# crabml/crabml

Measured on NVIDIA H100. Metric: decode_tokens_per_s, higher is better.
Workload: dtype int8

## Files before the change

crabml_b200/csrc/common.cuh:

```cuda
#pragma once

#include <cuda_fp16.h>
#include <cuda_runtime.h>
#include <stdint.h>

#include <atomic>
#include <map>
#include <mutex>
#include <set>
#include <string>
#include <unordered_map>
#include <vector>

#include "../../include/crabml_cuda.h"

#define QK_K 256

#define CC_D_STRIDE(nb) ((((nb) + 7) / 8) * 8)
#define CC_HAS_PADDED_D(t) ((t) == CC_Q8_0 || (t) == CC_Q4_0)
#define CC_MAX_PLANES 4
#define CC_N_SLOTS 16
#define CC_HISTORY_CAP 65536

struct cc_device;
// ... 182 lines not shown
    const uint8_t* p3[3];
    float* out[3];
    int m[3];
    int n;
};
struct StreamArgs {
    StreamMats mats;
    const void* act;
    int k;
    int epilogue;
    const float* residual;
    const uint16_t* exp_lut;
};
struct AttnArgs {
    const float *q, *k, *v;
    void *kcache, *vcache;
    float* out;
    void* act_scratch;
    const int64_t* dyn;
    const float* rope_tab;
    int n_heads, n_kv, hd, rope_dim, max_len, kv_f16;
    int64_t seq_stride;
    float scale;
};
struct DeqPlanes { const uint8_t* p[CC_MAX_PLANES]; int64_t cols; };
enum { MK_NORMQ = 0, MK_MATVEC = 1, MK_ATTN = 2, MK_ROWS = 3, MK_REDUCE = 4, MK_GATHER = 5, MK_ARGMAX = 6, MK_SAMPLE = 7 };
struct MkPhase {
    int type, wtype, write_back, next_matvec;
    int xgpu, red_n; const float* next_norm_w; float* red_dst; const float* red_res;
    float* x; float* orig; const float* norm_w; float eps; int n; ActQ8_0 act;
    int act_type, next_norm_n;
    StreamArgs mv;
    AttnArgs at;
    unsigned long long dyn_off, rope_off;
    DeqPlanes planes; int src_dtype, dst_dtype, n_rows, pad; long long cols; void* dst;
    const long long* rows_dev;
    long long* slot_dev; long long* hist_dev;
    int norm_ahead, pad2;
};
#define MK_PROF_SLOTS 9
size_t cc_mega_smem_for_phase(const MkPhase& ph);
const CommDev* cc_comm_dev(cc_device* dev);
bool cc_comm_is_nccl(cc_device* dev);
int cc_comm_world(cc_device* dev);
void cc_comm_destroy(cc_device* dev);
int cc_launch_all_reduce(cc_device* dev, float* x, int64_t n, const float* residual);
int cc_launch_all_gather(cc_device* dev, const float* src, int64_t n, float* dst);
extern "C" CC_API int cc_test_mega_barrier_floor(cc_device* dev, int n, float* us_per_phase);
enum MegaVariant { MEGA_NONE = 0, MEGA_REGISTER = 1, MEGA_RING = 2 };
struct MegaLaunch {
    MegaVariant variant = MEGA_NONE;
    size_t smem = 1024, wstage = 0;
    int slot_bytes = 0, nslots = 0, at_ch = 64;
    bool generic = false, sample = false;
};
int cc_launch_mega(cc_device* dev, const MkPhase* phases_dev, int n_phases, const uint8_t* dyn_dev, unsigned* bar_dev, const MegaLaunch& L,
                   unsigned long long* prof);
bool cc_mega_test_stall();
bool cc_mega_ring_phase_ok(const MkPhase& ph);
int cc_mega_ring_at_ch(const MkPhase& ph);
size_t cc_mega_ring_smem_for_phase(const MkPhase& ph);
int cc_mega_ring_slots(const MegaLaunch& L);
int cc_launch_mega_ring(cc_device* dev, const MkPhase* phases_dev, int n_phases, const uint8_t* dyn_dev, unsigned* bar_dev, const MegaLaunch& L,
                        unsigned long long* prof, const CommDev* comm);
int cc_check_async_error(cc_device* dev);
int cc_launch_normq(cc_device* dev, float* x, float* orig, const float* norm_w, float eps, int64_t n, void* act_scratch, bool write_back);
int cc_launch_attn_decode(cc_device* dev, const AttnArgs& a);
bool cc_attn_decode_fits(int64_t hd, int64_t max_len);
struct LazyState;
LazyState* cc_lazy_create(cc_device* dev);
void cc_lazy_destroy(cc_device* dev);
int cc_lazy_flush(cc_device* dev);
int cc_lazy_invalidate(cc_device* dev);
bool cc_stream_supported(int type, int64_t k);
bool cc_mega_generic_supported(int type, int64_t k);
int cc_launch_matvec_stream(cc_device* dev, int type, const StreamArgs& A);
int cc_launch_matvec_stream_plain(cc_device* dev, const cc_buf* w, const void* act, float* out, int64_t m, int64_t k);
// ... 90 lines not shown
```

crabml_b200/csrc/lazy.cu:

```cuda
#include <math.h>
#include <stdlib.h>
#include <string.h>

#include <chrono>
#include <functional>

#include "sample_dev.cuh"

enum LKind { L_COPY_ROWS, L_DUP, L_RMS_NORM, L_MUL, L_ADD, L_SCALE, L_MATVEC, L_ROPE, L_CONCAT, L_CONTIGUOUS, L_BMM, L_SOFTMAX, L_SILU, L_GELU, L_ALLREDUCE, L_ALLGATHER, L_ARGMAX, L_SAMPLE };

struct LView { cc_buf* buf = nullptr; int ndim = 0; int64_t shape[CC_MAX_DIMS] = {0, 0, 0, 0}, strides[CC_MAX_DIMS] = {0, 0, 0, 0}; };

struct LOp {
    int kind;
    LView a, b;
    cc_buf* out = nullptr;
    float f = 0.0f;
    int64_t i0 = 0, i1 = 0, i2 = 0;
    std::vector<int64_t> rows;
    bool done = false;
};

struct GraphEntry { cudaGraphExec_t exec = nullptr; size_t dyn_bytes = 0; uint64_t launches = 0; MkPhase* phases_dev = nullptr;
                    std::vector<uint64_t> sig; uint64_t last_use = 0; MegaVariant mega_variant = MEGA_NONE; };
#define LZ_MAX_GRAPHS 64

struct LazyState {
    std::vector<LOp> q;
    std::unordered_map<cc_buf*, int> qrefs;
#define LZ_DYN_SLOTS 8
    uint8_t* dyn_host[LZ_DYN_SLOTS] = {nullptr};
    cudaEvent_t dyn_ev[LZ_DYN_SLOTS] = {nullptr};
    int dyn_slot = 0;
    uint8_t* dyn_dev = nullptr;
    size_t dyn_cap = 1 << 16;
    void* act[2] = {nullptr, nullptr};
    unsigned* bar_dev = nullptr;
    unsigned long long* prof_dev = nullptr;
    std::vector<int> prof_types;
    size_t act_cap = 0;
    std::unordered_map<uint64_t, GraphEntry> cache;
    uint64_t flushes = 0, graph_hits = 0, captures = 0, uncached = 0, evictions = 0, collisions = 0;
    uint64_t ns_record = 0, ns_fuse = 0, ns_submit = 0, n_ops = 0;
    MegaVariant mega_variant = MEGA_NONE;
};

static LView mkview(const cc_view* v) {
    LView l;
    if (!v) return l;
    l.buf = v->buf; l.ndim = v->ndim;
    for (int i = 0; i < v->ndim; i++) { l.shape[i] = v->shape[i]; l.strides[i] = v->strides[i]; }
    return l;
}
static int64_t vlen(const LView& v) { int64_t n = 1; for (int i = 0; i < v.ndim; i++) n *= v.shape[i]; return n; }
static bool vcontig(const LView& v) {
    if (v.ndim == 0) return true;
    if (v.strides[v.ndim - 1] != 1) return false;
    int64_t last = 1;
    for (int i = v.ndim - 1; i >= 0; i--) { if (last != v.strides[i]) return false; last *= v.shape[i]; }
// ... 4 lines not shown
    if (ge.exec) cudaGraphExecDestroy(ge.exec);
    if (ge.phases_dev) cudaFree(ge.phases_dev);
    ge.exec = nullptr; ge.phases_dev = nullptr;
}
static void graph_cache_clear(LazyState* lz) {
    for (auto& kv : lz->cache) graph_entry_free(kv.second);
    lz->cache.clear();
}
int cc_lazy_invalidate(cc_device* dev) {
    LazyState* lz = dev->lz;
    if (!lz) return CC_OK;
    graph_cache_clear(lz);
    if (cudaMemsetAsync(lz->bar_dev, 0, 4096, dev->stream) != cudaSuccess) return cc_fail(dev, CC_ERR_CUDA, "lazy: barrier reset failed");
    return CC_OK;
}

LazyState* cc_lazy_create(cc_device* dev) {
    LazyState* lz = new LazyState();
    for (int i = 0; i < LZ_DYN_SLOTS; i++)
        if (cudaMallocHost(&lz->dyn_host[i], lz->dyn_cap) != cudaSuccess || cudaEventCreateWithFlags(&lz->dyn_ev[i], cudaEventDisableTiming) != cudaSuccess) { delete lz; return nullptr; }
    if (cudaMalloc(&lz->dyn_dev, lz->dyn_cap) != cudaSuccess) { delete lz; return nullptr; }
    if (getenv("CRABML_MEGA_PROF") && cudaMalloc(&lz->prof_dev, MK_PROF_SLOTS * 8 * 4097) == cudaSuccess) cudaMemset(lz->prof_dev, 0, MK_PROF_SLOTS * 8 * 4097);
    if (cudaMalloc(&lz->bar_dev, 4096) != cudaSuccess || cudaMemset(lz->bar_dev, 0, 4096) != cudaSuccess) { delete lz; return nullptr; }
    return lz;
}
void cc_lazy_destroy(cc_device* dev) {
    LazyState* lz = dev->lz;
    if (!lz) return;
    for (auto& op : lz->q) { if (op.a.buf) cc_tensor_release(op.a.buf); if (op.b.buf) cc_tensor_release(op.b.buf); if (op.out) cc_tensor_release(op.out); }
    for (auto& kv : lz->cache) graph_entry_free(kv.second);
    lz->cache.clear();
    if (lz->bar_dev) cudaFree(lz->bar_dev);
    for (int i = 0; i < LZ_DYN_SLOTS; i++) { if (lz->dyn_host[i]) cudaFreeHost(lz->dyn_host[i]); if (lz->dyn_ev[i]) cudaEventDestroy(lz->dyn_ev[i]); }
    if (lz->dyn_dev) cudaFree(lz->dyn_dev);
    for (int i = 0; i < 2; i++) if (lz->act[i]) cudaFree(lz->act[i]);
    delete lz;
    dev->lz = nullptr;
}

static void hold(LazyState* lz, cc_buf* b) { if (b) { cc_tensor_retain(b); lz->qrefs[b]++; } }

int cc_lazy_record(cc_device* dev, int kind, const cc_view* a, const cc_view* b, cc_buf* out, float f, int64_t i0, int64_t i1, int64_t i2,
                   const int64_t* rows, int n_rows) {
    LazyState* lz = dev->lz;
    auto t0 = std::chrono::steady_clock::now();
    LOp op;
    op.kind = kind; op.a = mkview(a); op.b = mkview(b); op.out = out; op.f = f; op.i0 = i0; op.i1 = i1; op.i2 = i2;
    if (rows) op.rows.assign(rows, rows + n_rows);
    hold(lz, op.a.buf); hold(lz, op.b.buf); hold(lz, op.out);
    lz->q.push_back(std::move(op));
    lz->n_ops++;
    lz->ns_record += (uint64_t)std::chrono::duration_cast<std::chrono::nanoseconds>(std::chrono::steady_clock::now() - t0).count();
    return CC_OK;
}

struct Plan {
    std::vector<uint64_t> sig;
    std::vector<uint8_t> dyn;
// ... 248 lines not shown
        if (!cc_attn_decode_fits(hd, seq_stride / hd)) return 0;
        if (!dead_after(ct.out, i + 9) || !dead_after(b1.out, i + 9) || !dead_after(qb, i + 9) || !dead_after(kb, i + 9) || !dead_after(vb, i + 9)) return 0;
        const int64_t pos = rq.i0, rope_dim = rq.rows[0];
        if (rope_dim > hd || rope_dim % 2) return 0;
        if (rope_off == (size_t)-1 || rope_pos != pos || rope_hd != hd || this->rope_dim != rope_dim) {
            std::vector<float> tab((size_t)rope_dim);
            const int pairs = (int)rope_dim / 2;
            float theta_scale = powf(10000.0f, -2.0f / (float)hd), theta = (float)pos;
            for (int j = 0; j < pairs; j++) { tab[j] = cosf(theta); tab[pairs + j] = sinf(theta); theta *= theta_scale; }
            rope_off = P.dyn_put(tab.data(), tab.size() * 4);
            rope_pos = pos; rope_hd = (int)hd; this->rope_dim = (int)rope_dim;
        }
        int64_t dynv[2] = {pos, kv_len};
        size_t dyn_off = P.dyn_put(dynv, sizeof(dynv));
        AttnArgs A = {};
        A.q = (const float*)qb->plane[0]; A.k = (const float*)kb->plane[0]; A.v = (const float*)vb->plane[0];
        A.kcache = kc->plane[0]; A.vcache = vc->plane[0];
        A.out = (float*)b2.out->base;
        if (*quantized && is(i + 9, L_MATVEC) && !cc_stream_supported(q[i + 9].a.buf->dtype, q[i + 9].a.shape[1])) *quantized = false;
        A.act_scratch = *quantized ? lz->act[1] : nullptr;
        A.n_heads = (int)n_heads; A.n_kv = (int)n_kv; A.hd = (int)hd; A.rope_dim = (int)rope_dim;
        A.max_len = (int)(seq_stride / hd); A.kv_f16 = kc->dtype == CC_F16;
        A.seq_stride = seq_stride; A.scale = sc.f;
        cc_device* d = dev;
        size_t roff = rope_off;
        P.S(0x2004); P.SP(A.q); P.SP(A.k); P.SP(A.v); P.SP(A.kcache); P.SP(A.vcache); P.SP(A.out); P.SP(A.act_scratch);
        P.S(n_heads); P.S(n_kv); P.S(hd); P.S(rope_dim); P.S(seq_stride); P.S(A.kv_f16); uint32_t sb; memcpy(&sb, &A.scale, 4); P.S(sb); P.S(dyn_off); P.S(roff);
        P.steps.push_back([=](uint8_t* dyn_dev) {
            AttnArgs B = A;
            B.dyn = (const int64_t*)(dyn_dev + dyn_off);
            B.rope_tab = (const float*)(dyn_dev + roff);
            return cc_launch_attn_decode(d, B);
        });
        { MkPhase ph = {}; ph.type = MK_ATTN; ph.at = A; ph.dyn_off = dyn_off; ph.rope_off = roff; ph.act = cc_act_q8_0(lz->act[1], n_heads * hd);
          P.phases.push_back(ph); }
        *obuf = b2.out;
        for (size_t t = i; t < i + 9; t++) q[t].done = true;
        return 9;
    }

    size_t try_copy_rows(size_t i) {
        if (!is(i, L_COPY_ROWS)) return 0;
        const LOp& op = q[i];
        cc_device* d = dev;
        const cc_buf* src = op.b.buf;
        void* dst = op.a.buf->plane[0];
        int dt = op.a.buf->dtype;
        int64_t cols = op.a.shape[op.a.ndim - 1];
        const int slot = (int)op.i2 - 1;
// ... 133 lines not shown
    }
};

static MegaLaunch choose_mega(const cc_device* dev, bool mega_ok, std::vector<MkPhase>& phs) {
    MegaLaunch L;
    if (!dev->mega || !mega_ok || phs.empty()) return L;
    bool stream = false, ring_ok = true;
    int n_sample = 0;
    for (auto& ph : phs) {
        if (ph.type == MK_MATVEC) (ph.act_type == CC_Q8_K ? L.generic : stream) = true;
        if (!cc_mega_ring_phase_ok(ph)) ring_ok = false;
        n_sample += ph.type == MK_SAMPLE;
    }
    L.sample = n_sample > 0;
    if (n_sample > 1 || (n_sample == 1 && phs.back().type != MK_SAMPLE)) return L;
    for (auto& ph : phs) {
        L.smem = std::max(L.smem, stream ? cc_mega_ring_smem_for_phase(ph) : cc_mega_smem_for_phase(ph));
        if (ph.type == MK_MATVEC && ph.x && ph.norm_w) L.wstage = std::max(L.wstage, (size_t)ph.n * 4);
        if (stream && ph.type == MK_MATVEC && ph.act_type != CC_Q8_K) L.slot_bytes = std::max(L.slot_bytes, ph.wtype == CC_Q8_0 ? 4352 : 2304);
        if (stream && ph.type == MK_ATTN) L.at_ch = cc_mega_ring_at_ch(ph);
    }
    if (stream ? !ring_ok || !(L.nslots = cc_mega_ring_slots(L)) : L.smem + L.wstage + 4096 > 227 * 1024) return L;
    L.variant = stream ? MEGA_RING : MEGA_REGISTER;
    int nxt = -1, nxn = -1;
    for (int t = (int)phs.size() - 1; t >= 0; t--) {
        MkPhase& ph = phs[t];
        ph.next_matvec = nxt;
        ph.next_norm_w = nxn >= 0 && phs[nxn].norm_ahead ? phs[nxn].norm_w : nullptr;
        ph.next_norm_n = ph.next_norm_w ? phs[nxn].n : 0;
        if (ph.type == MK_MATVEC) nxt = t;
        if (ph.type == MK_MATVEC && ph.x && ph.norm_w) nxn = t;
    }
    return L;
}

static int size_scratch(cc_device* dev, LazyState* lz) {
    int64_t max_k = 0;
    for (auto& op : lz->q) if (op.kind == L_MATVEC) max_k = std::max<int64_t>(max_k, std::max<int64_t>(op.a.shape[1], 0));
    for (auto& op : lz->q) if (op.kind == L_BMM && op.b.ndim == 3 && op.b.strides[2] == 1) max_k = std::max<int64_t>(max_k, op.a.shape[0] * op.b.shape[2]);
    size_t need = cc_act_bytes(CC_Q8_0, (max_k + 255) / 256 * 256) + 256;
    int rc = CC_OK;
    if (need > lz->act_cap) {
        cudaStreamSynchronize(dev->stream);
        graph_cache_clear(lz);
        for (int i = 0; i < 2; i++) { if (lz->act[i]) cudaFree(lz->act[i]); lz->act[i] = nullptr; }
        size_t cap = (size_t)1 << 20; while (cap < need) cap <<= 1;
        for (int i = 0; i < 2; i++) if (cudaMalloc(&lz->act[i], cap) != cudaSuccess) return cc_fail(dev, CC_ERR_CUDA, "lazy: scratch alloc failed");
        lz->act_cap = cap;
    }
    for (auto& op : lz->q) if (op.kind == L_MATVEC) {
        int at = cc_partner_type(op.a.buf->dtype);
        int64_t bb = op.b.ndim == 1 ? 1 : op.b.shape[0];
        if (at != CC_F32 && (rc = cc_ensure_act_scratch(dev, cc_act_bytes(at, bb * op.a.shape[1])))) return rc;
    }
    for (auto& op : lz->q) if (op.kind == L_SAMPLE && (rc = cc_ensure_sample_scratch(dev, vlen(op.a)))) return rc;
    return CC_OK;
}

static int upload_dyn(cc_device* dev, LazyState* lz, const Plan& P) {
    if (P.dyn.size() > lz->dyn_cap) return cc_fail(dev, CC_ERR_UNSUPPORTED, "lazy: dynamic argument block too large");
    if (P.dyn.empty()) return CC_OK;
    int rc = CC_OK; const int s = lz->dyn_slot;
    lz->dyn_slot = (s + 1) % LZ_DYN_SLOTS;
    cudaEventSynchronize(lz->dyn_ev[s]);
    memcpy(lz->dyn_host[s], P.dyn.data(), P.dyn.size());
    if (cudaMemcpyAsync(lz->dyn_dev, lz->dyn_host[s], P.dyn.size(), cudaMemcpyHostToDevice, dev->stream) != cudaSuccess) rc = cc_fail(dev, CC_ERR_CUDA, "lazy: dyn upload failed");
    cudaEventRecord(lz->dyn_ev[s], dev->stream);
    return rc;
}

static int run_steps(const Plan& P, uint8_t* dyn_dev) {
// ... 136 lines not shown
```

crabml_b200/csrc/mega.cu:

```cuda
#define MK_SYNC() __syncthreads()
#include "mega_phases.cuh"

struct MkNextNorm { const float* norm_w; int norm_n; };

template <bool SMP>
__global__ void __launch_bounds__(MK_THREADS, MK_CTAS_PER_SM) mega_kernel(const MkPhase* __restrict__ phases, int n_phases, const uint8_t* dyn,
                                                                         unsigned* bar, const uint16_t* exp_lut, unsigned long long* prof, bool test_stall, int wtop_off,
                                                                         unsigned* err_host) {
    extern __shared__ __align__(16) uint8_t smem[];
    __shared__ float s_red[MK_WARPS];
    __shared__ MkPhase s_phs[2];
    __shared__ MkNextNorm s_next;
    __shared__ int s_abort;
    __shared__ __align__(8) unsigned long long s_abar[AT_NBUF];
    unsigned apar = 0u;
    const unsigned abar0 = (unsigned)__cvta_generic_to_shared(&s_abar[0]);
    if (threadIdx.x == 0) { for (int i = 0; i < AT_NBUF; i++) mbar_init(abar0 + 8u * i, 1u); s_abort = 0; }
    asm volatile("fence.mbarrier_init.release.cluster;" ::: "memory");
    asm volatile("fence.proxy.async.shared::cta;" ::: "memory");
    __syncthreads();
    const CommDev nocomm = {};
    KSeg S0, S1;
    uint8_t* work = smem;
    float* s_w = (float*)(smem + wtop_off);
    int wstaged = -1;
    int xstaged = -1;
    unsigned gen = 0;
    if (threadIdx.x == MK_BAR_THREAD) gen = ld_acquire_u32(&bar[32]);
    {
        const int* src = (const int*)phases;
        int* dst = (int*)&s_phs[0];
// ... 9 lines not shown
        const int nx = s_ph.next_matvec;
        const bool look = nx > p && nx < n_phases;
        int desc_w = 0, next_w = 0;
        if (p + 1 < n_phases && threadIdx.x < sizeof(MkPhase) / 4) desc_w = ((const int*)(phases + p + 1))[threadIdx.x];
        if (look && threadIdx.x < 3) {
            const MkPhase* ph = phases + nx;
            next_w = threadIdx.x < 2 ? ((const int*)&ph->norm_w)[threadIdx.x] : ph->x && ph->norm_w && ph->norm_ahead ? ph->n : 0;
        }
        switch (s_ph.type) {
        case MK_NORMQ: phase_normq(s_ph, s_red); break;
        case MK_MATVEC: {
            unsigned long long* st1 = stamp ? prof + p * MK_PROF_SLOTS + 1 : nullptr;
            switch (s_ph.wtype) {
            case CC_Q2_K: phase_matvec_generic<TQ2_K>(s_ph, work, s_w, wstaged == p, xstaged == p, exp_lut, st1, S0, S1); break;
            case CC_Q3_K: phase_matvec_generic<TQ3_K>(s_ph, work, s_w, wstaged == p, xstaged == p, exp_lut, st1, S0, S1); break;
            case CC_Q4_K: phase_matvec_generic<TQ45_K<false>>(s_ph, work, s_w, wstaged == p, xstaged == p, exp_lut, st1, S0, S1); break;
            case CC_Q5_K: phase_matvec_generic<TQ45_K<true>>(s_ph, work, s_w, wstaged == p, xstaged == p, exp_lut, st1, S0, S1); break;
            case CC_Q6_K: phase_matvec_generic<TQ6_K>(s_ph, work, s_w, wstaged == p, xstaged == p, exp_lut, st1, S0, S1); break;
            default: phase_matvec_generic<TQ8_K>(s_ph, work, s_w, wstaged == p, xstaged == p, exp_lut, st1, S0, S1); break;
            }
            break;
        }
        case MK_ATTN:
            if (s_ph.at.kv_f16) phase_attn<true>(s_ph, (float*)work, s_red, dyn, exp_lut, abar0, apar, AT_CH); else phase_attn<false>(s_ph, (float*)work, s_red, dyn, exp_lut, abar0, apar, AT_CH);
            break;
        case MK_ROWS: phase_rows(s_ph, dyn); break;
        case MK_ARGMAX: phase_argmax(s_ph, dyn, s_red); break;
        }
        if (stamp) prof[p * MK_PROF_SLOTS + 2] = globaltimer_ns();
        if (p + 1 < n_phases && threadIdx.x < sizeof(MkPhase) / 4) ((int*)&s_phs[(p + 1) & 1])[threadIdx.x] = desc_w;
        if (look && threadIdx.x < 3) ((int*)&s_next)[threadIdx.x] = next_w;
        const bool more = p + 1 < n_phases;
        if (test_stall && p == 2 && blockIdx.x == gridDim.x - 1) { if (threadIdx.x == 0) s_abort = 1; break; }
        if (more) grid_barrier_arrive(bar, gridDim.x, gen);
        if (look && s_next.norm_n > 0) {
            const unsigned sw = (unsigned)__cvta_generic_to_shared(s_w);
            const float* nw = s_next.norm_w;
            for (int i = threadIdx.x; i < (s_next.norm_n >> 2); i += MK_THREADS)
                asm volatile("cp.async.cg.shared.global [%0], [%1], 16;" ::"r"(sw + i * 16), "l"(nw + i * 4) : "memory");
            asm volatile("cp.async.commit_group;" ::: "memory");
            wstaged = nx;
        }
        if (stamp) prof[p * MK_PROF_SLOTS + 3] = globaltimer_ns();
        if (more) {
            grid_barrier_wait(bar, gridDim.x, gen, nocomm, 0u, &s_abort, err_host);
            gen++;
            if (s_abort) break;
// ... 31 lines not shown
    CC_CUDA(dev, cudaMalloc(&d_tab, tab.size() * sizeof(MkPhase)));
    CC_CUDA(dev, cudaMalloc(&d_bar, 4096));
    CC_CUDA(dev, cudaMemcpy(d_tab, tab.data(), tab.size() * sizeof(MkPhase), cudaMemcpyHostToDevice));
    cudaEvent_t e0, e1;
    cudaEventCreate(&e0); cudaEventCreate(&e1);
    float best = 1e30f;
    for (int rep = 0; rep < 4; rep++) {
        CC_CUDA(dev, cudaMemsetAsync(d_bar, 0, 4096, dev->stream));
        cudaEventRecord(e0, dev->stream);
        MegaLaunch L;
        L.variant = MEGA_REGISTER;
        int rc = cc_launch_mega(dev, d_tab, n, nullptr, d_bar, L, nullptr);
        if (rc) return rc;
        cudaEventRecord(e1, dev->stream);
        CC_CUDA(dev, cudaEventSynchronize(e1));
        float ms = 0; cudaEventElapsedTime(&ms, e0, e1);
        if (ms < best) best = ms;
    }
    *us_per_phase = best * 1e3f / (float)n;
    cudaEventDestroy(e0); cudaEventDestroy(e1); cudaFree(d_tab); cudaFree(d_bar);
    return CC_OK;
}

bool cc_mega_generic_supported(int type, int64_t k) {
    return (type == CC_Q2_K || type == CC_Q3_K || type == CC_Q4_K || type == CC_Q5_K || type == CC_Q6_K || type == CC_Q8_K) && k % 256 == 0 && k <= 32768;
}

bool cc_mega_test_stall() {
    static const bool on = getenv("CRABML_MEGA_FLAGS") && (strtol(getenv("CRABML_MEGA_FLAGS"), nullptr, 0) & MK_F_TESTSTALL);
    return on;
}

int cc_launch_mega(cc_device* dev, const MkPhase* phases_dev, int n_phases, const uint8_t* dyn_dev, unsigned* bar_dev, const MegaLaunch& L,
                   unsigned long long* prof) {
    int max_ctas_per_sm = 0;
    const size_t wtop = (L.smem + 15) & ~(size_t)15;
    const size_t smem = wtop + L.wstage;
    CC_REQUIRE(dev, smem <= 227 * 1024, "megakernel: a phase needs %zu bytes of shared memory", smem);
    auto kern = L.sample ? mega_kernel<true> : mega_kernel<false>;
    if (smem > 48 * 1024) CC_CUDA(dev, cudaFuncSetAttribute(kern, cudaFuncAttributeMaxDynamicSharedMemorySize, (int)smem));
    CC_CUDA(dev, cudaOccupancyMaxActiveBlocksPerMultiprocessor(&max_ctas_per_sm, kern, MK_THREADS, smem));
    CC_REQUIRE(dev, max_ctas_per_sm >= 1, "megakernel does not fit on an SM");
    int per_sm = max_ctas_per_sm < MK_CTAS_PER_SM ? max_ctas_per_sm : MK_CTAS_PER_SM;
    const uint16_t* lut = dev->exp_lut;
    return mk_launch(dev, kern, dev->sm_count * per_sm, MK_THREADS, smem, phases_dev, n_phases, dyn_dev, bar_dev, lut, prof, cc_mega_test_stall(),
                     (int)wtop, dev->err_host);
}
```

crabml_b200/csrc/mega_phases.cuh:

```cuda
#pragma once
#include <stdlib.h>
#include <string.h>

#include "common.cuh"
#include "dequant.cuh"
#include "quantize_dev.cuh"
#include "vecdot.cuh"
#include "sample_dev.cuh"

#ifndef MK_SYNC
#error "define MK_SYNC() before including mega_phases.cuh"
#endif

#define MK_THREADS 512
#define MK_WARPS 16
#define MK_CTAS_PER_SM 1
#define MK_SEG 4
#define MK_XSTAGE_ROWS 512

__device__ __forceinline__ unsigned ld_acquire_u32(const unsigned* p) {
    unsigned v;
    asm volatile("ld.acquire.gpu.global.u32 %0, [%1];" : "=r"(v) : "l"(p) : "memory");
    return v;
}
// ... 234 lines not shown
        auto finish = [&]() { if (++c_seg < NSEG) return; c_seg = 0; const float v = warp_sum(acc); acc = 0.0f; emit(c_i++, v); };
        for (int u = 0; u < U; u += 2) {
            acc = T::seg_dot(S0, x0, k, c_seg, smem, lane, acc);
            finish();
            load(S0, x0, u + 2 < U);
            if (u + 1 >= U) break;
            acc = T::seg_dot(S1, x1, k, c_seg, smem, lane, acc);
            finish();
            load(S1, x1, u + 3 < U);
        }
    } else {
        for (int i = 0; i < n_vrows; i++) {
            int mat;
            const int r = locate(i, mat);
            emit(i, warp_sum(T::row_dot(planes(mat), r, k, smem, lane)));
        }
    }
    flush_pending();
}

#define AT_CH 64
#define AT_NBUF 3
template <bool KV_F16>
static __device__ void phase_attn(const MkPhase& ph, float* sm, float* s_red, const uint8_t* dyn, const uint16_t* exp_lut, unsigned abar0, unsigned& apar, const int at_ch) {
    const AttnArgs& a = ph.at;
    const int n_heads = a.n_heads, n_kv = a.n_kv, hd = a.hd, rope_dim = a.rope_dim;
    const int64_t seq_stride = a.seq_stride;
    const int64_t* dynv = (const int64_t*)(dyn + ph.dyn_off);
    const float* rope_tab = (const float*)(dyn + ph.rope_off);
    const int kv_len = (int)dynv[1], L = kv_len + 1;
    const int lane = threadIdx.x & 31, warp = threadIdx.x >> 5;
    float* s_q = sm; float* s_k = sm + hd; float* s_v = sm + 2 * hd; float* s_p = sm + 3 * hd;
    uint8_t* s_buf = (uint8_t*)(sm + 3 * hd + ((a.max_len + 8 + 3) & ~3));
    const unsigned s_buf_smem = (unsigned)__cvta_generic_to_shared(s_buf);
    constexpr int ELT = KV_F16 ? 2 : 4;
    const unsigned buf_bytes = (unsigned)(at_ch * hd * ELT);
    const int pairs = rope_dim >> 1;
    const int hd4 = hd >> 2;
    const int NC = (kv_len + at_ch - 1) / at_ch;
    auto issue_job = [&](int g, int j) {
        const int c = j < NC ? j : j - NC;
        const int p0 = c * at_ch, cnt = min(at_ch, kv_len - p0);
        const uint8_t* src = (const uint8_t*)(j < NC ? a.kcache : a.vcache) + ((int64_t)g * seq_stride + (int64_t)p0 * hd) * ELT;
        const unsigned bytes = (unsigned)(cnt * hd * ELT), bar = abar0 + 8u * (unsigned)(j % AT_NBUF), dst = s_buf_smem + (unsigned)(j % AT_NBUF) * buf_bytes;
        asm volatile("mbarrier.arrive.expect_tx.shared::cta.b64 _, [%0], %1;" ::"r"(bar), "r"(bytes) : "memory");
        asm volatile("cp.async.bulk.shared::cluster.global.mbarrier::complete_tx::bytes [%0], [%1], %2, [%3];" ::"r"(dst), "l"(src), "r"(bytes), "r"(bar) : "memory");
    };
// ... 101 lines not shown
            if (KV_F16) { acch = __hadd(acch, __hmul(__float2half_rn(s_v[d]), __float2half_rn(s_p[kv_len]))); o = __half2float(acch); }
            else { accf += s_p[kv_len] * s_v[d]; o = accf; }
            a.out[h * hd + d] = o;
            s_o[d] = o;
        }
        MK_SYNC();
        if (a.act_scratch) {
            ActQ8_0 act = ph.act;
            for (int b = warp; b < (hd >> 5); b += MK_WARPS) {
                float v = s_o[b * 32 + lane];
                float amax = warp_max(fabsf(v));
                float dd = amax / 127.0f;
                int qq = __float2int_rz(v / dd);
                const int gb = h * (hd >> 5) + b;
                act.qs[gb * 32 + lane] = (int8_t)qq;
                int ss = warp_sum_i(qq);
                if (lane == 0) { act.d[gb] = __half2float(__float2half_rn(dd)); act.isum[gb] = ss; }
            }
        }
        MK_SYNC();
    }
}

static __device__ void phase_rows(const MkPhase& ph, const uint8_t* dyn) {
    const int64_t* rows = ph.rows_dev ? (const int64_t*)ph.rows_dev : (const int64_t*)(dyn + ph.dyn_off);
    const int64_t total = (int64_t)ph.n_rows * ph.cols;
    for (int64_t i = (int64_t)blockIdx.x * MK_THREADS + threadIdx.x; i < total; i += (int64_t)gridDim.x * MK_THREADS) {
        const int64_t r = i / ph.cols, c = i - r * ph.cols;
        const int64_t e = rows[r] * ph.cols + c;
        float v;
        if (ph.src_dtype == CC_F32) v = __ldcg((const float*)ph.planes.p[0] + e);
        else if (ph.src_dtype == CC_F16) v = __half2float(((const __half*)ph.planes.p[0])[e]);
        else v = dequant_elem(ph.src_dtype, ph.planes, e);
        if (ph.dst_dtype == CC_F32) ((float*)ph.dst)[i] = v; else ((__half*)ph.dst)[i] = __float2half_rn(v);
    }
}

static __device__ void phase_argmax(const MkPhase& ph, const uint8_t* dyn, float* s_red) {
    if (blockIdx.x != 0) return;
    __shared__ long long s_idx[MK_WARPS];
    const float* x = ph.x;
    float bv = 0.0f; long long bi = -1;
    for (long long i = threadIdx.x; i < ph.n; i += MK_THREADS) { const float v = ldcg_f(x + i); if (bi < 0 || !(v < bv)) { bv = v; bi = i; } }
#pragma unroll
    for (int o = 16; o > 0; o >>= 1) {
        const float ov = __shfl_xor_sync(0xffffffffu, bv, o);
// ... 63 lines not shown
```

crabml_b200/csrc/mega_ring.cu:

```cuda
#define MK_SYNC() asm volatile("bar.sync 1, 512;" ::: "memory")
#define MK_GENERIC_NOINLINE 1
#include "mega_phases.cuh"

#define MR_PRODUCER_WARPS 4
#define MR_THREADS (MK_THREADS + 32 * MR_PRODUCER_WARPS)
#define MR_MAX_SLOTS 112
#define MR_Q8_SLOTS 24
#define MR_DESC_WORDS ((int)(sizeof(MkPhase) / 4))
#define MR_DESC_PER_LANE ((MR_DESC_WORDS + 31) / 32)

struct MrRing {
    int ring_off;
    int slot_bytes;
    int nslots;
    int at_ch;
};

__device__ __forceinline__ void mr_expect_tx(unsigned bar, unsigned bytes) { asm volatile("mbarrier.arrive.expect_tx.shared::cta.b64 _, [%0], %1;" ::"r"(bar), "r"(bytes) : "memory"); }
__device__ __forceinline__ void mr_bulk_g2s(unsigned dst, const void* src, unsigned bytes, unsigned bar, unsigned long long pol) {
    asm volatile("cp.async.bulk.shared::cluster.global.mbarrier::complete_tx::bytes.L2::cache_hint [%0], [%1], %2, [%3], %4;" ::"r"(dst), "l"(src), "r"(bytes), "r"(bar), "l"(pol) : "memory");
}
__device__ __forceinline__ void mr_stage_f32(float* dst, const float* src, int n) {
    const unsigned s = (unsigned)__cvta_generic_to_shared(dst);
    for (int i = threadIdx.x; i < (n >> 2); i += MK_THREADS) asm volatile("cp.async.cg.shared.global [%0], [%1], 16;" ::"r"(s + i * 16), "l"(src + i * 4) : "memory");
// ... 384 lines not shown
                    int mat;
                    const int rr = mr_locate(M, g, rc, 0, mat);
                    float* o = mat == 0 ? M.out[0] : mat == 1 ? M.out[1] : M.out[2];
                    o[rr] = r;
                }
            }
        }
    }
    flush_pending();
    if (stamp1) { stamp1[5] = (unsigned long long)c_wait; stamp1[6] = ((unsigned long long)(clock64() - c_all) << 20) | (unsigned long long)c_n; }
    RC.ent_base += (unsigned)(g.n_units * g.E);
    if (A.epilogue == 3) {
        MK_SYNC();
        if (warp < comm.world) {
            const size_t off = ((size_t)((xseq + 1u) & 1u) * CC_COMM_MAX_RANKS + comm.rank) * CC_COMM_MAX_ELEMS + g.first;
            for (int c4 = lane * 4; c4 < g.n_units; c4 += 128) *(float4*)(comm.data[warp] + off + c4) = *(const float4*)(s_part + c4);
        }
    }
}

template <bool GEN, bool SMP>
__global__ void __launch_bounds__(MR_THREADS, 1) mega_ring_kernel(const MkPhase* __restrict__ phases, int n_phases, const uint8_t* dyn, unsigned* bar,
                                                                  const uint16_t* exp_lut, unsigned long long* prof, bool test_stall, int wtop_off, unsigned* err_host,
                                                                  const CommDev comm, const MrRing R) {
    extern __shared__ __align__(128) uint8_t smem[];
    __shared__ float s_red[MK_WARPS];
    __shared__ MkPhase s_phs[2];
    __shared__ MkPhase s_pd[MR_PRODUCER_WARPS][2];
    __shared__ int s_abort;
    __shared__ int s_prod_done;
    __shared__ int s_ring_dead;
    __shared__ int s_unit;
    __shared__ __align__(8) unsigned long long s_abar[AT_NBUF];
    __shared__ __align__(8) unsigned long long s_full[MR_MAX_SLOTS];
    __shared__ unsigned s_done[MR_MAX_SLOTS];
    __shared__ unsigned s_seq[MR_MAX_SLOTS];
    unsigned apar = 0u;
    const unsigned abar0 = (unsigned)__cvta_generic_to_shared(&s_abar[0]);
    const unsigned full0 = (unsigned)__cvta_generic_to_shared(&s_full[0]);
    const unsigned done0 = (unsigned)__cvta_generic_to_shared(&s_done[0]);
    if (threadIdx.x == 0) {
        for (int i = 0; i < AT_NBUF; i++) mbar_init(abar0 + 8u * i, 1u);
        for (int i = 0; i < R.nslots; i++) { mbar_init(full0 + 8u * i, 1u); s_done[i] = 0u; s_seq[i] = 0u; }
        s_abort = 0; s_prod_done = 0; s_ring_dead = 0;
    }
    asm volatile("fence.mbarrier_init.release.cluster;" ::: "memory");
    asm volatile("fence.proxy.async.shared::cta;" ::: "memory");
// ... 24 lines not shown
        static_assert(sizeof(MkPhase) / 4 <= MK_THREADS, "descriptor does not fit one word per thread");
        int desc_w = 0;
        if (p + 1 < n_phases && threadIdx.x < sizeof(MkPhase) / 4) desc_w = ((const int*)(phases + p + 1))[threadIdx.x];
        unsigned long long* st1 = stamp ? prof + p * MK_PROF_SLOTS + 1 : nullptr;
        switch (s_ph.type) {
        case MK_NORMQ: phase_normq(s_ph, s_red); break;
        case MK_MATVEC:
            if (GEN && s_ph.act_type == CC_Q8_K) {
                switch (s_ph.wtype) {
                case CC_Q2_K: phase_matvec_generic<TQ2_K>(s_ph, work, s_wn, s_ph.norm_w == wst, false, exp_lut, st1); break;
                case CC_Q3_K: phase_matvec_generic<TQ3_K>(s_ph, work, s_wn, s_ph.norm_w == wst, false, exp_lut, st1); break;
                case CC_Q4_K: phase_matvec_generic<TQ45_K<false>>(s_ph, work, s_wn, s_ph.norm_w == wst, false, exp_lut, st1); break;
                case CC_Q5_K: phase_matvec_generic<TQ45_K<true>>(s_ph, work, s_wn, s_ph.norm_w == wst, false, exp_lut, st1); break;
                case CC_Q6_K: phase_matvec_generic<TQ6_K>(s_ph, work, s_wn, s_ph.norm_w == wst, false, exp_lut, st1); break;
                default: phase_matvec_generic<TQ8_K>(s_ph, work, s_wn, s_ph.norm_w == wst, false, exp_lut, st1); break;
                }
                if (s_ph.x && s_ph.norm_w) { wst = s_ph.next_norm_w; if (wst) mr_stage_f32(s_wn, wst, s_ph.next_norm_n); }
                break;
            }
            if (s_ph.wtype == CC_Q8_0) phase_matvec_ring<CC_Q8_0>(s_ph, work, s_wn, wst, xstaged == p, exp_lut, RC, comm, xseq, st1);
            else phase_matvec_ring<CC_Q4_0>(s_ph, work, s_wn, wst, xstaged == p, exp_lut, RC, comm, xseq, st1);
            break;
        case MK_ATTN:
            if (s_ph.at.kv_f16) phase_attn<true>(s_ph, (float*)work, s_red, dyn, exp_lut, abar0, apar, R.at_ch);
            else phase_attn<false>(s_ph, (float*)work, s_red, dyn, exp_lut, abar0, apar, R.at_ch);
            break;
        case MK_ROWS: phase_rows(s_ph, dyn); break;
        case MK_REDUCE: phase_reduce(s_ph, comm, xseq, false); break;
        case MK_GATHER: phase_reduce(s_ph, comm, xseq, true); break;
        case MK_ARGMAX: phase_argmax(s_ph, dyn, s_red); break;
        }
        if (stamp) prof[p * MK_PROF_SLOTS + 2] = globaltimer_ns();
        if (p + 1 < n_phases && threadIdx.x < sizeof(MkPhase) / 4) ((int*)&s_phs[(p + 1) & 1])[threadIdx.x] = desc_w;
        const bool more = p + 1 < n_phases;
        const bool xg = s_ph.xgpu != 0;
        if (test_stall && p == 2 && blockIdx.x == gridDim.x - 1) { if (threadIdx.x == 0) s_abort = 1; break; }
        if (more) grid_barrier_arrive(bar, gridDim.x, gen);
        if (stamp) prof[p * MK_PROF_SLOTS + 3] = globaltimer_ns();
        if (more) {
            grid_barrier_wait(bar, gridDim.x, gen, comm, xg ? xseq + 1u : 0u, &s_abort, err_host);
            gen++; if (xg) xseq++;
            if (s_abort) break;
            const MkPhase& nph = s_phs[(p + 1) & 1];
            if (nph.type == MK_MATVEC && nph.act_type != CC_Q8_K && nph.x && !nph.red_n) { mr_stage_f32((float*)(work + mr_x_off(nph.mv.k)), nph.x, nph.mv.k); xstaged = p + 1; }
        }
    }
    asm volatile("cp.async.wait_all;" ::: "memory");
    if constexpr (SMP) {
// ... 42 lines not shown
    if (L.slot_bytes <= 0 || off >= cap) return 0;
    const int fit = (int)std::min((cap - off) / (size_t)L.slot_bytes, (size_t)MR_MAX_SLOTS);
    if (fit < MR_MIN_SLOTS) return 0;
    return L.slot_bytes >= 4352 ? std::min(fit, MR_Q8_SLOTS) : fit;
}

int cc_launch_mega_ring(cc_device* dev, const MkPhase* phases_dev, int n_phases, const uint8_t* dyn_dev, unsigned* bar_dev, const MegaLaunch& L,
                        unsigned long long* prof, const CommDev* comm) {
    auto kern = mr_kernel(L);
    const size_t wtop = (L.smem + 15) & ~(size_t)15;
    const size_t ring_off = mr_ring_off(L);
    const size_t smem = ring_off + (size_t)L.nslots * L.slot_bytes;
    CC_CUDA(dev, cudaFuncSetAttribute(kern, cudaFuncAttributeMaxDynamicSharedMemorySize, (int)smem));
    int max_ctas_per_sm = 0;
    CC_CUDA(dev, cudaOccupancyMaxActiveBlocksPerMultiprocessor(&max_ctas_per_sm, kern, MR_THREADS, smem));
    CC_REQUIRE(dev, max_ctas_per_sm >= 1, "megakernel (ring) does not fit on an SM");
    CommDev cd;
    memset(&cd, 0, sizeof(cd));
    if (comm) cd = *comm;
    MrRing R;
    R.ring_off = (int)ring_off; R.slot_bytes = L.slot_bytes; R.nslots = L.nslots; R.at_ch = L.at_ch;
    const uint16_t* lut = dev->exp_lut;
    return mk_launch(dev, kern, dev->sm_count, MR_THREADS, smem, phases_dev, n_phases, dyn_dev, bar_dev, lut, prof, cc_mega_test_stall(), (int)wtop,
                     dev->err_host, (const CommDev)cd, (const MrRing)R);
}
```

Baseline: 279.7.

## Split decode attention per head across multiple CTAs with global score exchange

Adds a split-KV attention path in the megakernel. Each head is spread over up to four CTAs: each computes QK scores for its slice of positions, writes them to a global scratch buffer, and synchronizes with its peers through per-head atomic arrival counters. Each CTA then runs the full softmax and computes a slice of the head dimensions of the V product. The aim is to use more SMs when there are few heads and long contexts. The cost is an extra inter-CTA spin wait, global score traffic, redundant softmax work in every CTA, and a new scratch allocation.

```diff
diff --git a/crabml_b200/csrc/common.cuh b/crabml_b200/csrc/common.cuh
--- a/crabml_b200/csrc/common.cuh
+++ b/crabml_b200/csrc/common.cuh
@@ -228,7 +228,13 @@
     int n_heads, n_kv, hd, rope_dim, max_len, kv_f16;
     int64_t seq_stride;
     float scale;
-};
+    int split;
+};
+#define AT_SPLIT_MAX 4
+#define AT_SPLIT_MIN_KV 320
+#define AT_ARRIVE_WORD 128
+#define AT_SPLIT_MAX_HEADS ((1024 - AT_ARRIVE_WORD) / 8)
+int cc_attn_split(const AttnArgs& a, int grid);
 struct DeqPlanes { const uint8_t* p[CC_MAX_PLANES]; int64_t cols; };
 enum { MK_NORMQ = 0, MK_MATVEC = 1, MK_ATTN = 2, MK_ROWS = 3, MK_REDUCE = 4, MK_GATHER = 5, MK_ARGMAX = 6, MK_SAMPLE = 7 };
 struct MkPhase {
@@ -259,6 +265,7 @@
     size_t smem = 1024, wstage = 0;
     int slot_bytes = 0, nslots = 0, at_ch = 64;
     bool generic = false, sample = false;
+    float* scores = nullptr;
 };
 int cc_launch_mega(cc_device* dev, const MkPhase* phases_dev, int n_phases, const uint8_t* dyn_dev, unsigned* bar_dev, const MegaLaunch& L,
                    unsigned long long* prof);
diff --git a/crabml_b200/csrc/lazy.cu b/crabml_b200/csrc/lazy.cu
--- a/crabml_b200/csrc/lazy.cu
+++ b/crabml_b200/csrc/lazy.cu
@@ -35,6 +35,8 @@
     uint8_t* dyn_dev = nullptr;
     size_t dyn_cap = 1 << 16;
     void* act[2] = {nullptr, nullptr};
+    float* scores = nullptr;
+    size_t scores_cap = 0;
     unsigned* bar_dev = nullptr;
     unsigned long long* prof_dev = nullptr;
     std::vector<int> prof_types;
@@ -85,6 +87,8 @@
     if (cudaMalloc(&lz->dyn_dev, lz->dyn_cap) != cudaSuccess) { delete lz; return nullptr; }
     if (getenv("CRABML_MEGA_PROF") && cudaMalloc(&lz->prof_dev, MK_PROF_SLOTS * 8 * 4097) == cudaSuccess) cudaMemset(lz->prof_dev, 0, MK_PROF_SLOTS * 8 * 4097);
     if (cudaMalloc(&lz->bar_dev, 4096) != cudaSuccess || cudaMemset(lz->bar_dev, 0, 4096) != cudaSuccess) { delete lz; return nullptr; }
+    lz->scores_cap = (size_t)1 << 20;
+    if (cudaMalloc(&lz->scores, lz->scores_cap) != cudaSuccess) { delete lz; return nullptr; }
     return lz;
 }
 void cc_lazy_destroy(cc_device* dev) {
@@ -97,6 +101,7 @@
     for (int i = 0; i < LZ_DYN_SLOTS; i++) { if (lz->dyn_host[i]) cudaFreeHost(lz->dyn_host[i]); if (lz->dyn_ev[i]) cudaEventDestroy(lz->dyn_ev[i]); }
     if (lz->dyn_dev) cudaFree(lz->dyn_dev);
     for (int i = 0; i < 2; i++) if (lz->act[i]) cudaFree(lz->act[i]);
+    if (lz->scores) cudaFree(lz->scores);
     delete lz;
     dev->lz = nullptr;
 }
@@ -391,9 +396,10 @@
         A.n_heads = (int)n_heads; A.n_kv = (int)n_kv; A.hd = (int)hd; A.rope_dim = (int)rope_dim;
         A.max_len = (int)(seq_stride / hd); A.kv_f16 = kc->dtype == CC_F16;
         A.seq_stride = seq_stride; A.scale = sc.f;
+        A.split = (size_t)n_heads * (size_t)(A.max_len + 1) * 4 <= lz->scores_cap ? AT_SPLIT_MAX : 1;
         cc_device* d = dev;
         size_t roff = rope_off;
-        P.S(0x2004); P.SP(A.q); P.SP(A.k); P.SP(A.v); P.SP(A.kcache); P.SP(A.vcache); P.SP(A.out); P.SP(A.act_scratch);
+        P.S(0x2004); P.SP(A.q); P.SP(A.k); P.SP(A.v); P.SP(A.kcache); P.SP(A.vcache); P.SP(A.out); P.SP(A.act_scratch); P.S(A.split); P.SP(lz->scores);
         P.S(n_heads); P.S(n_kv); P.S(hd); P.S(rope_dim); P.S(seq_stride); P.S(A.kv_f16); uint32_t sb; memcpy(&sb, &A.scale, 4); P.S(sb); P.S(dyn_off); P.S(roff);
         P.steps.push_back([=](uint8_t* dyn_dev) {
             AttnArgs B = A;
@@ -573,6 +579,8 @@
     }
     if (stream ? !ring_ok || !(L.nslots = cc_mega_ring_slots(L)) : L.smem + L.wstage + 4096 > 227 * 1024) return L;
     L.variant = stream ? MEGA_RING : MEGA_REGISTER;
+    for (auto& ph : phs) if (ph.type == MK_ATTN) ph.at.split = cc_attn_split(ph.at, dev->sm_count);
+    L.scores = dev->lz->scores;
     int nxt = -1, nxn = -1;
     for (int t = (int)phs.size() - 1; t >= 0; t--) {
         MkPhase& ph = phs[t];
@@ -598,6 +606,18 @@
         size_t cap = (size_t)1 << 20; while (cap < need) cap <<= 1;
         for (int i = 0; i < 2; i++) if (cudaMalloc(&lz->act[i], cap) != cudaSuccess) return cc_fail(dev, CC_ERR_CUDA, "lazy: scratch alloc failed");
         lz->act_cap = cap;
+    }
+    size_t score_need = 0;
+    for (auto& op : lz->q)
+        if (op.kind == L_BMM && op.b.ndim == 3 && op.b.strides[1] == 1 && op.b.strides[2] > 0 && op.b.strides[0] > 0)
+            score_need = std::max(score_need, (size_t)op.a.shape[0] * (size_t)(op.b.strides[0] / op.b.strides[2] + 1) * 4);
+    if (score_need > lz->scores_cap) {
+        cudaStreamSynchronize(dev->stream);
+        graph_cache_clear(lz);
+        cudaFree(lz->scores); lz->scores = nullptr; lz->scores_cap = 0;
+        size_t cap = (size_t)1 << 20; while (cap < score_need) cap <<= 1;
+        if (cudaMalloc(&lz->scores, cap) != cudaSuccess) return cc_fail(dev, CC_ERR_CUDA, "lazy: score scratch alloc failed");
+        lz->scores_cap = cap;
     }
     for (auto& op : lz->q) if (op.kind == L_MATVEC) {
         int at = cc_partner_type(op.a.buf->dtype);
diff --git a/crabml_b200/csrc/mega.cu b/crabml_b200/csrc/mega.cu
--- a/crabml_b200/csrc/mega.cu
+++ b/crabml_b200/csrc/mega.cu
@@ -6,7 +6,7 @@
 template <bool SMP>
 __global__ void __launch_bounds__(MK_THREADS, MK_CTAS_PER_SM) mega_kernel(const MkPhase* __restrict__ phases, int n_phases, const uint8_t* dyn,
                                                                          unsigned* bar, const uint16_t* exp_lut, unsigned long long* prof, bool test_stall, int wtop_off,
-                                                                         unsigned* err_host) {
+                                                                         unsigned* err_host, float* scores) {
     extern __shared__ __align__(16) uint8_t smem[];
     __shared__ float s_red[MK_WARPS];
     __shared__ MkPhase s_phs[2];
@@ -62,7 +62,8 @@
             break;
         }
         case MK_ATTN:
-            if (s_ph.at.kv_f16) phase_attn<true>(s_ph, (float*)work, s_red, dyn, exp_lut, abar0, apar, AT_CH); else phase_attn<false>(s_ph, (float*)work, s_red, dyn, exp_lut, abar0, apar, AT_CH);
+            if (s_ph.at.kv_f16) phase_attn<true>(s_ph, (float*)work, s_red, dyn, exp_lut, abar0, apar, AT_CH, bar, err_host, &s_abort, scores);
+            else phase_attn<false>(s_ph, (float*)work, s_red, dyn, exp_lut, abar0, apar, AT_CH, bar, err_host, &s_abort, scores);
             break;
         case MK_ROWS: phase_rows(s_ph, dyn); break;
         case MK_ARGMAX: phase_argmax(s_ph, dyn, s_red); break;
@@ -140,6 +141,13 @@
     return CC_OK;
 }
 
+int cc_attn_split(const AttnArgs& a, int grid) {
+    if (a.split <= 1 || a.n_heads > AT_SPLIT_MAX_HEADS) return 1;
+    for (int S = AT_SPLIT_MAX; S > 1; S >>= 1)
+        if (a.hd % (32 * S) == 0 && a.n_heads * S <= grid) return S;
+    return 1;
+}
+
 bool cc_mega_generic_supported(int type, int64_t k) {
     return (type == CC_Q2_K || type == CC_Q3_K || type == CC_Q4_K || type == CC_Q5_K || type == CC_Q6_K || type == CC_Q8_K) && k % 256 == 0 && k <= 32768;
 }
@@ -162,5 +170,5 @@
     int per_sm = max_ctas_per_sm < MK_CTAS_PER_SM ? max_ctas_per_sm : MK_CTAS_PER_SM;
     const uint16_t* lut = dev->exp_lut;
     return mk_launch(dev, kern, dev->sm_count * per_sm, MK_THREADS, smem, phases_dev, n_phases, dyn_dev, bar_dev, lut, prof, cc_mega_test_stall(),
-                     (int)wtop, dev->err_host);
+                     (int)wtop, dev->err_host, L.scores);
 }
diff --git a/crabml_b200/csrc/mega_phases.cuh b/crabml_b200/csrc/mega_phases.cuh
--- a/crabml_b200/csrc/mega_phases.cuh
+++ b/crabml_b200/csrc/mega_phases.cuh
@@ -280,7 +280,7 @@
 #define AT_CH 64
 #define AT_NBUF 3
 template <bool KV_F16>
-static __device__ void phase_attn(const MkPhase& ph, float* sm, float* s_red, const uint8_t* dyn, const uint16_t* exp_lut, unsigned abar0, unsigned& apar, const int at_ch) {
+static __device__ void phase_attn_one(const MkPhase& ph, float* sm, float* s_red, const uint8_t* dyn, const uint16_t* exp_lut, unsigned abar0, unsigned& apar, const int at_ch) {
     const AttnArgs& a = ph.at;
     const int n_heads = a.n_heads, n_kv = a.n_kv, hd = a.hd, rope_dim = a.rope_dim;
     const int64_t seq_stride = a.seq_stride;
@@ -428,6 +428,212 @@
     }
 }
 
+#if MK_GENERIC_NOINLINE
+#define MK_ATTN_SPLIT_ATTR __noinline__
+#else
+#define MK_ATTN_SPLIT_ATTR
+#endif
+__device__ __forceinline__ unsigned atom_add_release(unsigned* p, unsigned v) {
+    unsigned old;
+    asm volatile("atom.release.gpu.global.add.u32 %0, [%1], %2;" : "=r"(old) : "l"(p), "r"(v) : "memory");
+    return old;
+}
+template <bool KV_F16>
+static __device__ MK_ATTN_SPLIT_ATTR void phase_attn_split(const MkPhase& ph, float* sm, float* s_red, const uint8_t* dyn, const uint16_t* exp_lut, unsigned abar0, unsigned& apar, const int at_ch,
+                                        unsigned* bar, unsigned* err_host, int* s_abort, float* scores) {
+    const AttnArgs& a = ph.at;
+    const int n_heads = a.n_heads, n_kv = a.n_kv, hd = a.hd, rope_dim = a.rope_dim, S = a.split;
+    const int64_t seq_stride = a.seq_stride;
+    const int64_t* dynv = (const int64_t*)(dyn + ph.dyn_off);
+    const float* rope_tab = (const float*)(dyn + ph.rope_off);
+    const int kv_len = (int)dynv[1], L = kv_len + 1;
+    const int lane = threadIdx.x & 31, warp = threadIdx.x >> 5;
+    float* s_q = sm; float* s_k = sm + hd; float* s_v = sm + 2 * hd; float* s_p = sm + 3 * hd;
+    uint8_t* s_buf = (uint8_t*)(sm + 3 * hd + ((a.max_len + 8 + 3) & ~3));
+    const unsigned s_buf_smem = (unsigned)__cvta_generic_to_shared(s_buf);
+    constexpr int ELT = KV_F16 ? 2 : 4;
+    const unsigned buf_bytes = (unsigned)(at_ch * hd * ELT);
+    const int pairs = rope_dim >> 1;
+    const int dw = hd / S, vch = at_ch * S;
+    const int NCV = (kv_len + vch - 1) / vch;
+    for (int u = blockIdx.x; u < n_heads * S; u += gridDim.x) {
+        const int h = u % n_heads, part = u / n_heads;
+        const int g = KV_F16 ? h / (n_heads / n_kv) : h % n_kv;
+        const int p_lo = (int)((int64_t)part * L / S), p_hi = (int)((int64_t)(part + 1) * L / S), k_hi = min(p_hi, kv_len);
+        const int NCK = k_hi > p_lo ? (k_hi - p_lo + at_ch - 1) / at_ch : 0;
+        const int NJ = NCK + NCV;
+        int v_issued = 0;
+        auto issue_job = [&](int j) {
+            const unsigned mb = abar0 + 8u * (unsigned)(j % AT_NBUF), dst = s_buf_smem + (unsigned)(j % AT_NBUF) * buf_bytes;
+            if (j < NCK) {
+                const int p0 = p_lo + j * at_ch, cnt = min(at_ch, k_hi - p0);
+                if (threadIdx.x == 0) {
+                    const uint8_t* src = (const uint8_t*)a.kcache + ((int64_t)g * seq_stride + (int64_t)p0 * hd) * ELT;
+                    const unsigned bytes = (unsigned)(cnt * hd * ELT);
+                    asm volatile("mbarrier.arrive.expect_tx.shared::cta.b64 _, [%0], %1;" ::"r"(mb), "r"(bytes) : "memory");
+                    asm volatile("cp.async.bulk.shared::cluster.global.mbarrier::complete_tx::bytes [%0], [%1], %2, [%3];" ::"r"(dst), "l"(src), "r"(bytes), "r"(mb) : "memory");
+                }
+            } else {
+                const int p0 = (j - NCK) * vch, cnt = min(vch, kv_len - p0), pr = dw * ELT / 16;
+                const uint8_t* src = (const uint8_t*)a.vcache + ((int64_t)g * seq_stride + (int64_t)p0 * hd + part * dw) * ELT;
+                for (int i = threadIdx.x; i < cnt * pr; i += MK_THREADS) {
+                    const int r = i / pr, q = i - r * pr;
+                    asm volatile("cp.async.cg.shared.global [%0], [%1], 16;" ::"r"(dst + (unsigned)(r * pr + q) * 16u), "l"(src + (int64_t)r * hd * ELT + q * 16) : "memory");
+                }
+                asm volatile("cp.async.commit_group;" ::: "memory");
+                v_issued++;
+            }
+        };
+        auto wait_job = [&](int j) {
+            if (j >= NCK) {
+                const int newer = v_issued - (j - NCK) - 1;
+                if (newer >= 2) asm volatile("cp.async.wait_group 2;" ::: "memory");
+                else if (newer == 1) asm volatile("cp.async.wait_group 1;" ::: "memory");
+                else asm volatile("cp.async.wait_group 0;" ::: "memory");
+                MK_SYNC();
+                return;
+            }
+            const int bsel = j % AT_NBUF;
+            mbar_wait(abar0 + 8u * (unsigned)bsel, (apar >> bsel) & 1u);
+            apar ^= 1u << bsel;
+        };
+        auto ld_kv = [&](const uint8_t* buf, int idx) -> float { return KV_F16 ? __half2float(((const __half*)buf)[idx]) : ((const float*)buf)[idx]; };
+        for (int j = 0; j < min(AT_NBUF, NJ); j++) issue_job(j);
+        for (int i = threadIdx.x; i < hd; i += MK_THREADS) {
+            float qv, kvv;
+            if (i < rope_dim) {
+                const int j = i >> 1;
+                const float c = rope_tab[j], s = rope_tab[pairs + j];
+                const float q0 = ldcg_f(a.q + h * hd + 2 * j), q1 = ldcg_f(a.q + h * hd + 2 * j + 1);
+                const float k0 = ldcg_f(a.k + g * hd + 2 * j), k1 = ldcg_f(a.k + g * hd + 2 * j + 1);
+                qv = (i & 1) ? q0 * s + q1 * c : q0 * c - q1 * s;
+                kvv = (i & 1) ? k0 * s + k1 * c : k0 * c - k1 * s;
+            } else {
+                qv = ldcg_f(a.q + h * hd + i);
+                kvv = ldcg_f(a.k + g * hd + i);
+            }
+            s_q[i] = qv * a.scale;
+            s_k[i] = kvv;
+            s_v[i] = ldcg_f(a.v + g * hd + i);
+        }
+        MK_SYNC();
+        const bool owner = part == 0 && (KV_F16 ? (h % (n_heads / n_kv) == 0) : (h < n_kv));
+        if (owner) {
+            for (int i = threadIdx.x; i < hd; i += MK_THREADS) {
+                const int64_t off = (int64_t)g * seq_stride + (int64_t)kv_len * hd + i;
+                if (KV_F16) { ((__half*)a.kcache)[off] = __float2half_rn(s_k[i]); ((__half*)a.vcache)[off] = __float2half_rn(s_v[i]); }
+                else { ((float*)a.kcache)[off] = s_k[i]; ((float*)a.vcache)[off] = s_v[i]; }
+            }
+        }
+        float* srow = scores + (size_t)h * (size_t)(a.max_len + 1);
+        for (int j = 0; j < NCK; j++) {
+            const int p0 = p_lo + j * at_ch, cnt = min(at_ch, k_hi - p0);
+            const uint8_t* kb = s_buf + (size_t)(j % AT_NBUF) * buf_bytes;
+            wait_job(j);
+            for (int s = warp; s < cnt; s += MK_WARPS) {
+                float acc = 0.0f;
+                for (int i = lane; i < hd; i += 32) acc += (KV_F16 ? __half2float(__float2half_rn(s_q[i])) : s_q[i]) * ld_kv(kb, s * hd + i);
+                acc = warp_sum(acc);
+                if (lane == 0) { s_p[p0 + s] = acc; srow[p0 + s] = acc; }
+            }
+            MK_SYNC();
+            if (j + AT_NBUF < NJ) issue_job(j + AT_NBUF);
+        }
+        if (warp == 0 && p_hi == L) {
+            float acc = 0.0f;
+            for (int i = lane; i < hd; i += 32) {
+                if (KV_F16) acc += __half2float(__float2half_rn(s_q[i])) * __half2float(__float2half_rn(s_k[i]));
+                else acc += s_q[i] * s_k[i];
+            }
+            acc = warp_sum(acc);
+            if (lane == 0) { s_p[kv_len] = acc; srow[kv_len] = acc; }
+        }
+        MK_SYNC();
+        {
+            if (threadIdx.x == 0) {
+                unsigned* w = bar + AT_ARRIVE_WORD + 8 * h;
+                const unsigned old = atom_add_release(w, AT_SPLIT_MAX / S), target = (old & ~(unsigned)(AT_SPLIT_MAX - 1)) + AT_SPLIT_MAX;
+                MkSpin sp;
+                for (unsigned v = old + AT_SPLIT_MAX / S; (int)(v - target) < 0; v = ld_acquire_u32(w))
+                    if (sp.expired(bar, err_host, 1u)) { *s_abort = 1; break; }
+            }
+            MK_SYNC();
+            for (int s = threadIdx.x; s < L; s += MK_THREADS) if (s < p_lo || s >= p_hi) s_p[s] = ldcg_f(srow + s);
+            MK_SYNC();
+        }
+        float m = -INFINITY;
+        for (int s = threadIdx.x; s < L; s += MK_THREADS) m = fmaxf(m, s_p[s]);
+        m = warp_max(m);
+        if (lane == 0) s_red[warp] = m;
+        MK_SYNC();
+        m = s_red[0];
+#pragma unroll
+        for (int w = 1; w < MK_WARPS; w++) m = fmaxf(m, s_red[w]);
+        MK_SYNC();
+        float sum = 0.0f;
+        for (int s = threadIdx.x; s < L; s += MK_THREADS) {
+            float e = h2f_bits(exp_lut[f2h_bits(s_p[s] - m)]);
+            s_p[s] = e;
+            sum += e;
+        }
+        sum = warp_sum(sum);
+        if (lane == 0) s_red[warp] = sum;
+        MK_SYNC();
+        sum = 0.0f;
+#pragma unroll
+        for (int w = 0; w < MK_WARPS; w++) sum += s_red[w];
+        for (int s = threadIdx.x; s < L; s += MK_THREADS) s_p[s] = s_p[s] / sum;
+        MK_SYNC();
+        float accf = 0.0f;
+        __half acch = __float2half_rn(0.0f);
+        const int t = threadIdx.x, d = part * dw + t;
+        for (int j = NCK; j < NJ; j++) {
+            const int p0 = (j - NCK) * vch, cnt = min(vch, kv_len - p0);
+            const uint8_t* vb = s_buf + (size_t)(j % AT_NBUF) * buf_bytes;
+            wait_job(j);
+            if (t < dw) {
+                for (int s = 0; s < cnt; s++) {
+                    if (KV_F16) acch = __hadd(acch, __hmul(((const __half*)vb)[s * dw + t], __float2half_rn(s_p[p0 + s])));
+                    else accf += s_p[p0 + s] * ((const float*)vb)[s * dw + t];
+                }
+            }
+            MK_SYNC();
+            if (j + AT_NBUF < NJ) issue_job(j + AT_NBUF);
+        }
+        float* s_o = s_k;
+        MK_SYNC();
+        if (t < dw) {
+            float o;
+            if (KV_F16) { acch = __hadd(acch, __hmul(__float2half_rn(s_v[d]), __float2half_rn(s_p[kv_len]))); o = __half2float(acch); }
+            else { accf += s_p[kv_len] * s_v[d]; o = accf; }
+            a.out[h * hd + d] = o;
+            s_o[t] = o;
+        }
+        MK_SYNC();
+        if (a.act_scratch) {
+            ActQ8_0 act = ph.act;
+            for (int b = warp; b < (dw >> 5); b += MK_WARPS) {
+                float v = s_o[b * 32 + lane];
+                float amax = warp_max(fabsf(v));
+                float dd = amax / 127.0f;
+                int qq = __float2int_rz(v / dd);
+                const int gb = h * (hd >> 5) + part * (dw >> 5) + b;
+                act.qs[gb * 32 + lane] = (int8_t)qq;
+                int ss = warp_sum_i(qq);
+                if (lane == 0) { act.d[gb] = __half2float(__float2half_rn(dd)); act.isum[gb] = ss; }
+            }
+        }
+        MK_SYNC();
+    }
+}
+
+template <bool KV_F16>
+static __device__ __forceinline__ void phase_attn(const MkPhase& ph, float* sm, float* s_red, const uint8_t* dyn, const uint16_t* exp_lut, unsigned abar0, unsigned& apar,
+                                                  const int at_ch, unsigned* bar, unsigned* err_host, int* s_abort, float* scores) {
+    if (ph.at.split > 1 && ((const int64_t*)(dyn + ph.dyn_off))[1] >= AT_SPLIT_MIN_KV) phase_attn_split<KV_F16>(ph, sm, s_red, dyn, exp_lut, abar0, apar, at_ch, bar, err_host, s_abort, scores);
+    else phase_attn_one<KV_F16>(ph, sm, s_red, dyn, exp_lut, abar0, apar, at_ch);
+}
+
 static __device__ void phase_rows(const MkPhase& ph, const uint8_t* dyn) {
     const int64_t* rows = ph.rows_dev ? (const int64_t*)ph.rows_dev : (const int64_t*)(dyn + ph.dyn_off);
     const int64_t total = (int64_t)ph.n_rows * ph.cols;
diff --git a/crabml_b200/csrc/mega_ring.cu b/crabml_b200/csrc/mega_ring.cu
--- a/crabml_b200/csrc/mega_ring.cu
+++ b/crabml_b200/csrc/mega_ring.cu
@@ -430,7 +430,7 @@
 template <bool GEN, bool SMP>
 __global__ void __launch_bounds__(MR_THREADS, 1) mega_ring_kernel(const MkPhase* __restrict__ phases, int n_phases, const uint8_t* dyn, unsigned* bar,
                                                                   const uint16_t* exp_lut, unsigned long long* prof, bool test_stall, int wtop_off, unsigned* err_host,
-                                                                  const CommDev comm, const MrRing R) {
+                                                                  const CommDev comm, const MrRing R, float* scores) {
     extern __shared__ __align__(128) uint8_t smem[];
     __shared__ float s_red[MK_WARPS];
     __shared__ MkPhase s_phs[2];
@@ -501,8 +501,8 @@
             else phase_matvec_ring<CC_Q4_0>(s_ph, work, s_wn, wst, xstaged == p, exp_lut, RC, comm, xseq, st1);
             break;
         case MK_ATTN:
-            if (s_ph.at.kv_f16) phase_attn<true>(s_ph, (float*)work, s_red, dyn, exp_lut, abar0, apar, R.at_ch);
-            else phase_attn<false>(s_ph, (float*)work, s_red, dyn, exp_lut, abar0, apar, R.at_ch);
+            if (s_ph.at.kv_f16) phase_attn<true>(s_ph, (float*)work, s_red, dyn, exp_lut, abar0, apar, R.at_ch, bar, err_host, &s_abort, scores);
+            else phase_attn<false>(s_ph, (float*)work, s_red, dyn, exp_lut, abar0, apar, R.at_ch, bar, err_host, &s_abort, scores);
             break;
         case MK_ROWS: phase_rows(s_ph, dyn); break;
         case MK_REDUCE: phase_reduce(s_ph, comm, xseq, false); break;
@@ -591,5 +591,5 @@
     R.ring_off = (int)ring_off; R.slot_bytes = L.slot_bytes; R.nslots = L.nslots; R.at_ch = L.at_ch;
     const uint16_t* lut = dev->exp_lut;
     return mk_launch(dev, kern, dev->sm_count, MR_THREADS, smem, phases_dev, n_phases, dyn_dev, bar_dev, lut, prof, cc_mega_test_stall(), (int)wtop,
-                     dev->err_host, (const CommDev)cd, (const MrRing)R);
-}
+                     dev->err_host, (const CommDev)cd, (const MrRing)R, L.scores);
+}
```

Measured after the change: 288.9, median of 6. 1.03x the previous value.
